# Jimmy2027/MoPoE-MIMIC

Hardware: AMD Instinct MI355X
Metric: samples/sec (higher is better)
Workload: dtype f32; 1 GPU; BASELINE config c2: MoPoE joint-ELBO train step, 3 modalities (PA+Lateral+text) 128x128, class_dim 128, DIM_img 64, DIM_text 128, vocab 3517, batch 64/GPU, fp32 (storage, accumulation and every product; where the launch plan says so the fp32 products are formed on the bf16 matrix pipe from exact three-way splits of both operands -- closer to fp64 than the fp32 MFMA, tests: test_f32_products_on_the; global_batch=64, parallelism=dp1, hip_graph=True, cross_rank_elbo=mean

## Files before the change

include/mopoe_hip.h:

```cpp
#ifndef MOPOE_HIP_H
#define MOPOE_HIP_H

#include <stddef.h>
#include <stdint.h>

#ifdef __cplusplus
extern "C" {
#endif

#define MOPOE_ABI_VERSION 23

#define MOPOE_OK 0
#define MOPOE_ERR_ARG (-1)
#define MOPOE_ERR_LAUNCH (-2)
#define MOPOE_ERR_DEVICE (-3)

int mopoe_abi_version(void);
const char* mopoe_last_error(void);

typedef struct {
  int32_t N;
  int32_t Hs, Ws;
  int32_t Hb, Wb;
  int32_t Cin, Cout;
// ... 150 lines not shown
                               const mopoe_mask_ref* mask1, const double* sums2, double* sums1, float* dw1, float* dbias,
                               float* dgamma2, float* dbeta2, void* stream);
int mopoe_block_front_stats(const float* x, const float* w1, const float* bias, int64_t rows, int32_t C,
                            const mopoe_bn_ref* bn1, const mopoe_mask_ref* mask1, double* stats_d1, void* stream);
int mopoe_block_front_apply(const float* x, const float* w1, const float* bias, float* a2, int64_t rows, int32_t C,
                            const mopoe_bn_ref* bn1, const mopoe_bn_ref* bn2, const mopoe_mask_ref* mask1, void* stream);
int mopoe_block_front_bwd(const float* x, const float* dh2, const float* w1, const float* bias, float* dh1, int64_t rows, int32_t C,
                          const mopoe_bn_ref* bn1, const mopoe_bn_ref* bn2, const mopoe_mask_ref* mask1, const double* sums2,
                          double* sums1, float* dw1, float* dbias, float* dgamma2, float* dbeta2, void* stream);
int mopoe_lse_rows(const void* logits, int32_t is_bf16, int64_t rows, int32_t V, float* lse, void* stream);
int mopoe_token_nll_logits_fwd(const void* logits, int32_t is_bf16, const float* lse, const float* ids, int64_t rows, int32_t V,
                               float norm, float* out, double* ws, void* stream);
int mopoe_token_softmax_grad_logits(const void* logits, int32_t is_bf16, const float* lse, const float* ids, const float* g,
                                    int64_t rows, int32_t V, float norm, void* dx, void* stream);
int mopoe_dense_logprob_rows(const float* logp, const float* target, int64_t rows, int64_t per_row,
                             int64_t target_rows, float* out, void* stream);

int mopoe_lhood_style_sample(const float* mu, const float* logvar, const float* eps, const float* style_mu,
                             const float* style_logvar, const float* style_eps, int32_t K, int32_t B, int32_t D, int32_t S,
                             float* zcat, float* t_c, float* t_s, void* stream);
int mopoe_lhood_estimates(const float* const lp[3], const float* t_c, const float* t_s, int32_t K, int32_t B,
                          int32_t subset_mask, float* out, void* stream);

int mopoe_logreg_fit(const float* X, const float* Y, int32_t S, int32_t N, int32_t D, int32_t L, float C, int32_t max_iter,
                     float tol, float* W, float* info, void* stream);
int mopoe_logreg_predict(const float* const* x, int32_t S, int32_t M, int32_t D, int32_t L, const float* W, float* pred,
                         float* dec, void* stream);

int mopoe_embedding_fwd(const float* ids, const float* table, float* out, int64_t rows, int32_t V,
                        int32_t D, void* stream);
int mopoe_embedding_bwd(const float* ids, const float* gout, float* dtable, int64_t rows, int32_t V,
                        int32_t D, int32_t padding_idx, void* stream);


int mopoe_conv_fwd_bf16(const uint16_t* x, const uint16_t* wp, const float* bias, void* y, int32_t y_is_f32,
                        const mopoe_conv_geom* g, const mopoe_bn_ref* bn_in, const mopoe_mask_ref* mask,
                        double* out_stats, const mopoe_conv_plan* plan, void* workspace, size_t workspace_bytes,
                        void* stream);
int mopoe_conv_fwd_mix_bf16(const uint16_t* x, const uint16_t* wp, const float* bias, uint16_t* y,
                            const mopoe_conv_geom* g, const mopoe_bn_ref* bn_in, const mopoe_mask_ref* mask,
                            const mopoe_mix_ref* mix, double* out_stats, const mopoe_conv_plan* plan, void* workspace,
                            size_t workspace_bytes, void* stream);
int mopoe_conv_dgrad_bf16(const uint16_t* dy, const uint16_t* wp, void* dx, int32_t dx_is_f32, const mopoe_conv_geom* g,
                          const mopoe_bn_ref* relu_bn, const uint16_t* xin, double* bwd_sums,
                          const mopoe_conv_plan* plan, void* workspace, size_t workspace_bytes, void* stream);
int mopoe_conv_wgrad_bf16(const uint16_t* x, const uint16_t* dy, float* dwp, const mopoe_conv_geom* g,
                          const mopoe_bn_ref* bn_in, int32_t dwp_is_zero, const mopoe_conv_plan* plan, void* stream);
int mopoe_edge_expand_bf16(const float* scal, const float* w, uint16_t* out, const mopoe_conv_geom* g, int32_t C,
                           double* stats, void* stream);
int mopoe_edge_wgrad_bf16(const uint16_t* vec, const float* scal, float* dw, const mopoe_conv_geom* g, int32_t C,
                          int32_t dw_is_zero, void* stream);
int mopoe_edge_reduce_bf16(const uint16_t* x, const float* w, const float* bias, float* out, const mopoe_conv_geom* g,
                           int32_t C, void* stream);
int mopoe_bn_relu_apply_bf16(const uint16_t* x, uint16_t* out, int64_t rows, int32_t C, const mopoe_bn_ref* bn, void* stream);
int mopoe_block_out_fwd_bf16(const uint16_t* s, const uint16_t* m, uint16_t* out, int64_t rows, int32_t C,
                             const mopoe_bn_ref* bn_s, float a, float b, double* out_stats, void* stream);
int mopoe_bn_bwd_reduce_bf16(const uint16_t* g, const uint16_t* s, int64_t rows, int32_t C, const mopoe_bn_ref* bn_s,
                             double* sums, void* stream);
int mopoe_block_out_bwd_bf16(const uint16_t* g, const uint16_t* s, uint16_t* dm, uint16_t* ds, int64_t rows, int32_t C,
                             const mopoe_bn_ref* bn_s, const double* sums, const mopoe_mask_ref* mask, float a, float b,
                             float* dgamma, float* dbeta, float* colsum_dm, float* colsum_ds, void* stream);
int mopoe_bn_bwd_apply_bf16(const uint16_t* dy, const uint16_t* x, const uint16_t* add, uint16_t* dx, int64_t rows,
                            int32_t C, const mopoe_bn_ref* bn, const double* sums, const mopoe_mask_ref* mask,
                            float* dgamma, float* dbeta, float* colsum_dx, const uint16_t* next_s,
                            const mopoe_bn_ref* next_bn, double* next_sums, void* stream);
int mopoe_colsum_bf16(const uint16_t* x, float* out, int64_t rows, int32_t C, int32_t out_is_zero, void* stream);
int mopoe_logsoftmax_bwd_bf16out(const float* dy, const float* y, uint16_t* dx, int64_t rows, int32_t V, void* stream);
int mopoe_embedding_fwd_bf16(const float* ids, const float* table, uint16_t* out, int64_t rows, int32_t V, int32_t D,
                             void* stream);
int mopoe_embedding_bwd_bf16(const float* ids, const uint16_t* gout, float* dtable, int64_t rows, int32_t V, int32_t D,
                             int32_t padding_idx, void* stream);

typedef struct {
  float* p;
  const float* g;
  float* m;
  float* v;
  uint16_t* p16;
  int64_t n;
} mopoe_adam_seg;
int mopoe_adam_step(const mopoe_adam_seg* segs, int32_t nseg, float* step, const float* lr_dev, double lr, double beta1,
                    double beta2, double eps, float* coef, void* stream);

#define MOPOE_PROF_KINDS 144
int mopoe_prof_enable(int32_t on);
int mopoe_prof_stamp(uint64_t* slot, void* stream);
int mopoe_prof_collect(int64_t* launches, double* total_ms, double* total_flops, double* total_bytes );

#ifdef __cplusplus
}
#endif
#endif
```

mopoe-mimic_amd/csrc/conv_gemm.hip:

```cpp
#include "gemm_common.hpp"

namespace mopoe {

constexpr int BK = 16;
#ifndef TILE_N64_REMAINDER
#define TILE_N64_REMAINDER 64
#endif
#ifndef SPLIT_BLOCKS
#define SPLIT_BLOCKS 256
#endif
#ifndef SPLIT_TARGET
#define SPLIT_TARGET 512
#endif
#ifndef GEMM_8WAVES
#define GEMM_8WAVES 1
#endif
#ifndef PERSIST_BLOCKS
#define PERSIST_BLOCKS 2048
#endif
#ifndef GEMM_MIN_WAVES
#define GEMM_MIN_WAVES 3
#endif
#ifndef GEMM_BK_BIG
#define GEMM_BK_BIG 16
#endif
#ifndef GEMM_LDS_PAD
#define GEMM_LDS_PAD 4
#endif
constexpr int LDS_PAD = GEMM_LDS_PAD;

struct GemmArgs {
  const float* X;
  const float* W;
  float* Y;
  const float* bias;
  int N, Hx, Wx, Hy, Wy, Ck, Cn, Cin_w, Cout_w;
  int kh, kw, sh, sw, ph, pw;
  int form, w_nk;
  int Hq, Wq;
  long rows_per_phase;
  int vecA, vecB;
  mopoe_bn_ref bn_in;
  mopoe_mask_ref mask;
  double* out_stats;
  mopoe_bn_ref relu_bn;
  const float* xin;
  double* bwd_sums;
  unsigned x_bytes, w_bytes;
  int nsplit;
  float* partial;
  int* counters;
  long rows_total;
  int mix;
  float mix_a, mix_b;
  int xcd_remap;
};

__device__ __forceinline__ float epi_round(const GemmArgs&, float x) { return x; }
struct EpiXinRaw { float4 lo, hi; };
constexpr bool EPI_PREFETCH_XIN = false;
__device__ __forceinline__ EpiXinRaw epi_xin_ld(const GemmArgs& a, long yrow, int ncol, bool ok_hi) {
  const float* p = a.xin + yrow * a.Cn + ncol;
  EpiXinRaw r;
  r.lo = *reinterpret_cast<const float4*>(p);
  r.hi = ok_hi ? *reinterpret_cast<const float4*>(p + 4) : make_float4(0.f, 0.f, 0.f, 0.f);
  return r;
}
__device__ __forceinline__ void epi_xin_unpack(const EpiXinRaw& r, float (&xi)[8]) {
  xi[0] = r.lo.x; xi[1] = r.lo.y; xi[2] = r.lo.z; xi[3] = r.lo.w; xi[4] = r.hi.x; xi[5] = r.hi.y; xi[6] = r.hi.z; xi[7] = r.hi.w;
}
__device__ __forceinline__ void epi_store8(const GemmArgs& a, long yrow, int ncol, bool ok_hi, const float (&v)[8]) {
  float* dst = a.Y + yrow * a.Cn + ncol;
  *reinterpret_cast<float4*>(dst) = make_float4(v[0], v[1], v[2], v[3]);
  if (ok_hi) *reinterpret_cast<float4*>(dst + 4) = make_float4(v[4], v[5], v[6], v[7]);
}


__device__ __forceinline__ float4 bld4(__amdgpu_buffer_rsrc_t srd, unsigned byte_off) {
  const u32x4 v = __builtin_amdgcn_raw_buffer_load_b128(srd, byte_off, 0, 0);
  return make_float4(__uint_as_float(v.x), __uint_as_float(v.y), __uint_as_float(v.z), __uint_as_float(v.w));
}

// ... 1092 lines not shown
    return edge_expand(x, wp, y, g, g->Cout, out_stats, (hipStream_t)stream);
  if (plain && g->transposed && g->Cout == 1 && !out_stats && edge_supported(g, g->Cin, {x, wp}))
    return edge_reduce(x, wp, bias, y, g, g->Cin, (hipStream_t)stream);
  return launch_gather(x, wp, bias, y, g, g->transposed ? 0 : 1, g->Cin, g->Cout, 0, bn_in, mask, out_stats,
                       nullptr, nullptr, nullptr, plan, workspace, workspace_bytes, (hipStream_t)stream);
}

extern "C" int mopoe_conv_fwd_mix(const float* x, const float* wp, const float* bias, float* y, const mopoe_conv_geom* g,
                                  const mopoe_bn_ref* bn_in, const mopoe_mask_ref* mask, const mopoe_mix_ref* mix,
                                  double* out_stats, const mopoe_conv_plan* plan, void* workspace, size_t workspace_bytes,
                                  void* stream) {
  if (int rc = validate_geom(g)) return rc;
  if (!x || !wp || !y || !mix) { set_error("conv_fwd_mix: null pointer"); return MOPOE_ERR_ARG; }
  return launch_gather(x, wp, bias, y, g, g->transposed ? 0 : 1, g->Cin, g->Cout, 0, bn_in, mask, out_stats,
                       nullptr, nullptr, nullptr, plan, workspace, workspace_bytes, (hipStream_t)stream, mix);
}

extern "C" int mopoe_conv_dgrad(const float* dy, const float* wp, float* dx, const mopoe_conv_geom* g,
                                const mopoe_bn_ref* relu_bn, const float* xin, double* bwd_sums,
                                const mopoe_conv_plan* plan, void* workspace, size_t workspace_bytes, void* stream) {
  if (int rc = validate_geom(g)) return rc;
  if (!dy || !wp || !dx) { set_error("conv_dgrad: null pointer"); return MOPOE_ERR_ARG; }
  if (g->transposed && g->Cout == 1 && (!relu_bn || relu_bn->mode == 0) && edge_supported(g, g->Cin, {wp, dx}))
    return edge_expand(dy, wp, dx, g, g->Cin, nullptr, (hipStream_t)stream);
  return launch_gather(dy, wp, nullptr, dx, g, g->transposed ? 1 : 0, g->Cout, g->Cin, 1, nullptr, nullptr,
                       nullptr, relu_bn, xin, bwd_sums, plan, workspace, workspace_bytes, (hipStream_t)stream);
}

extern "C" int mopoe_conv_wgrad(const float* x, const float* dy, float* dwp, const mopoe_conv_geom* g,
                                const mopoe_bn_ref* bn_in, int32_t dwp_is_zero, const mopoe_conv_plan* plan,
                                void* stream_) {
  if (int rc = validate_geom(g)) return rc;
  if (!x || !dy || !dwp) { set_error("conv_wgrad: null pointer"); return MOPOE_ERR_ARG; }
  hipStream_t stream = (hipStream_t)stream_;
  if ((!bn_in || bn_in->mode == 0) && !g->transposed && g->Cin == 1 && edge_supported(g, g->Cout, {dy, dwp}))
    return edge_wgrad(dy, x, dwp, g, g->Cout, stream, dwp_is_zero != 0);
  if ((!bn_in || bn_in->mode == 0) && g->transposed && g->Cout == 1 && edge_supported(g, g->Cin, {x, dwp}))
    return edge_wgrad(x, dy, dwp, g, g->Cin, stream, dwp_is_zero != 0);
  WgradArgs a;
  a.Xs = x; a.Dy = dy; a.dW = dwp;
  a.N = g->N; a.Hs = g->Hs; a.Ws = g->Ws; a.Hb = g->Hb; a.Wb = g->Wb; a.Cin = g->Cin; a.Cout = g->Cout;
  a.kh = g->kh; a.kw = g->kw; a.sh = g->sh; a.sw = g->sw; a.ph = g->ph; a.pw = g->pw;
  a.x_is_big = g->transposed ? 0 : 1;
  a.Ms = (long)g->N * g->Hs * g->Ws;
  mopoe_bn_ref none = {};
  a.bn_in = bn_in ? *bn_in : none;
  if (a.bn_in.mode != 0 && (a.bn_in.C != g->Cin || g->Cin > MAX_BN_C)) { set_error("wgrad bn_in channel mismatch"); return MOPOE_ERR_ARG; }
  a.vecI = (g->Cin % 4 == 0) && aligned16(x);
  a.vecJ = (g->Cout % 4 == 0) && aligned16(dy);
  const size_t rows_x = (size_t)g->N * (g->transposed ? g->Hs * g->Ws : g->Hb * g->Wb);
  const size_t rows_dy = (size_t)g->N * (g->transposed ? g->Hb * g->Wb : g->Hs * g->Ws);
  const size_t xb = rows_x * g->Cin * sizeof(float), db = rows_dy * g->Cout * sizeof(float);
  const bool vec = a.vecI && a.vecJ && xb < (1ull << 31) && db < (1ull << 31);
  a.x_bytes = (unsigned)std::min<size_t>(xb, 0x7fffffffu);
  a.dy_bytes = (unsigned)std::min<size_t>(db, 0x7fffffffu);
  if (rows_x >= (1ull << 31) || rows_dy >= (1ull << 31)) { set_error("wgrad: more than 2^31 rows"); return MOPOE_ERR_ARG; }
  const int hw_s = g->Hs * g->Ws;
  a.fast = (vec && ((g->Ws % BK == 0) || (BK % g->Ws == 0 && hw_s % BK == 0))) ? 1 : 0;
  const int taps = g->kh * g->kw;
  bool big = g->Cin > 64 && g->Cout > 64;
  if (plan && (plan->tile == 9 || plan->tile == 10)) {
    const bool ok = a.bn_in.mode == 0 && vec && g->kh == 4 && g->kw == 4 && g->sh == 2 && g->sw == 2 && g->ph == 1 && g->pw == 1 &&
                    g->Hs % 8 == 0 && g->Ws % 8 == 0 && g->Hb == 2 * g->Hs && g->Wb == 2 * g->Ws;
    if (!ok) {
      set_error("wgrad plan: tiles 9 / 10 (four taps per block) need a plain operand, the vector path, k4 s2 p1 and a small grid of whole 8 x 8 tiles");
      return MOPOE_ERR_ARG;
    }
    const int Cg = a.x_is_big ? g->Cin : g->Cout, Csm = a.x_is_big ? g->Cout : g->Cin;
    const int cs = plan->tile == 10 ? 128 : 64;
    if (cs == 128 && Csm % 128 != 0) { set_error("wgrad plan: tile 10 needs a multiple of 128 channels on the small-grid operand (%d)", Csm); return MOPOE_ERR_ARG; }
    const long ntiles = (long)g->N * (g->Hs / 8) * (g->Ws / 8);
    const long cblocks = (long)ceil_div(Cg, 64) * ceil_div(Csm, cs) * 4;
    long split = plan->split > 0 ? plan->split : (256 + cblocks - 1) / cblocks;
    if (split > ntiles) split = ntiles;
    if (split < 1) split = 1;
    a.chunk = (ntiles + split - 1) / split;
    split = (ntiles + a.chunk - 1) / a.chunk;
    a.atomic = split > 1;
    static const bool xcd_remap9 = !getenv("MOPOE_NO_XCD_REMAP");
    a.xcd_remap = xcd_remap9 ? 1 : 0;
    if (a.atomic && !dwp_is_zero) {
      if (hipMemsetAsync(dwp, 0, (size_t)taps * g->Cin * g->Cout * sizeof(float), stream) != hipSuccess) { set_error("wgrad memset failed"); return MOPOE_ERR_LAUNCH; }
    }
    ProfScope prof(stream, 2.0 * (double)a.Ms * g->Cin * (double)g->Cout * taps, PROF_F32_WGRAD_PARITY + (cs == 128 ? 2 : 0) + (a.x_is_big ? 0 : 1), (double)xb + (double)db);
    const dim3 grid((unsigned)(ceil_div(Cg, 64) * ceil_div(Csm, cs)), 4, (unsigned)split);
    if (cs == 128 && a.x_is_big) hipLaunchKernelGGL((wgrad_parity_f32_kernel<128, true>), grid, dim3(256), 0, stream, a);
    else if (cs == 128) hipLaunchKernelGGL((wgrad_parity_f32_kernel<128, false>), grid, dim3(256), 0, stream, a);
    else if (a.x_is_big) hipLaunchKernelGGL((wgrad_parity_f32_kernel<64, true>), grid, dim3(256), 0, stream, a);
    else hipLaunchKernelGGL((wgrad_parity_f32_kernel<64, false>), grid, dim3(256), 0, stream, a);
    return check_launch("wgrad_parity_f32 (four taps per block)");
  }
  const bool wemu = plan && (plan->tile == 7 || plan->tile == 8);
  if (wemu && a.bn_in.mode != 0) { set_error("wgrad plan: tile %d (split-bf16 products) has no BN-on-load form", plan->tile); return MOPOE_ERR_ARG; }
  if (plan && (plan->tile == 2 || plan->tile == 6 || plan->tile == 8)) big = false;
  else if (plan && (plan->tile == 5 || plan->tile == 7)) {
    if (!big) { set_error("wgrad plan: tile %d (128x128 on LDS-DMA) needs more than 64 channels on both sides (%d, %d)", plan->tile, g->Cin, g->Cout); return MOPOE_ERR_ARG; }
  }
  else if (plan && plan->tile > 2) { set_error("wgrad plan: tile %d (see mopoe_conv_plan in mopoe_hip.h: -1, 0, 2, 5, 6, 7, 8, 9, 10)", plan->tile); return MOPOE_ERR_ARG; }
  const bool glds = plan && plan->tile >= 5;
  if (glds && !vec) { set_error("wgrad plan: the LDS-DMA tiles need the vector path (channel counts %% 4 == 0, aligned tensors)"); return MOPOE_ERR_ARG; }
  const int T = big ? 128 : 64;
  const int nI = ceil_div(g->Cin, T), nJ = ceil_div(g->Cout, T);
  a.nJ = nJ;
  const long tiles = (long)nI * nJ * taps;
  long split = (1024 + tiles - 1) / tiles;
  if (plan && plan->split > 0) split = plan->split;
  const int kp = glds ? 32 : BK;
  const long max_split = glds ? (a.Ms + 4 * kp - 1) / (4 * kp) : (a.Ms + 8 * BK - 1) / (8 * BK);
  if (split > max_split) split = max_split;
  if (split < 1) split = 1;
  long chunk = (a.Ms + split - 1) / split;
  chunk = (chunk + kp - 1) / kp * kp;
  split = (a.Ms + chunk - 1) / chunk;
  a.chunk = chunk;
  a.atomic = split > 1;
  static const bool xcd_remap = !getenv("MOPOE_NO_XCD_REMAP");
  a.xcd_remap = xcd_remap ? 1 : 0;
  const size_t bytes = (size_t)taps * g->Cin * g->Cout * sizeof(float);
  if (a.atomic && !dwp_is_zero) {
    if (hipMemsetAsync(dwp, 0, bytes, stream) != hipSuccess) { set_error("wgrad memset failed"); return MOPOE_ERR_LAUNCH; }
  }
  const double flops = 2.0 * (double)a.Ms * g->Cin * (double)g->Cout * taps;
  const int spec = a.fast ? (a.bn_in.mode != 0 ? 2 : 1) : 0;
  const double abytes = ((double)g->N * g->Hs * g->Ws * (g->transposed ? g->Cin : g->Cout)
                         + (double)g->N * g->Hb * g->Wb * (g->transposed ? g->Cout : g->Cin)) * sizeof(float);
  ProfScope prof(stream, flops, wemu ? PROF_F32_WGRAD_GLDS_EMU + (big ? 0 : 1)
                                : glds ? PROF_F32_WGRAD_GLDS + (big ? 0 : 2) + (a.bn_in.mode != 0 ? 1 : 0)
                                     : (vec ? PROF_WGRAD_VEC + (big ? 0 : 3) + spec : PROF_WGRAD_SCALAR + (big ? 0 : 1)), abytes);
  dim3 grid(nI * nJ, taps, (unsigned)split);
  if (wemu) {
    if (big) hipLaunchKernelGGL((wgrad_gemm_f32_glds_kernel<128, false, 2, 1>), grid, dim3(256), 0, stream, a);
    else hipLaunchKernelGGL((wgrad_gemm_f32_glds_kernel<64, false, 4, 1>), grid, dim3(256), 0, stream, a);
  } else if (glds) {
    const bool xf = a.bn_in.mode != 0;
    if (big) {
      if (xf) hipLaunchKernelGGL((wgrad_gemm_f32_glds_kernel<128, true, 2>), grid, dim3(256), 0, stream, a);
      else hipLaunchKernelGGL((wgrad_gemm_f32_glds_kernel<128, false, 2>), grid, dim3(256), 0, stream, a);
    } else {
      if (xf) hipLaunchKernelGGL((wgrad_gemm_f32_glds_kernel<64, true, 2>), grid, dim3(256), 0, stream, a);
      else hipLaunchKernelGGL((wgrad_gemm_f32_glds_kernel<64, false, 4>), grid, dim3(256), 0, stream, a);
    }
  } else if (vec) {
    if (big) {
      if (spec == 1) hipLaunchKernelGGL((wgrad_gemm_kernel<128, 128, true, 1>), grid, dim3(256), 0, stream, a);
      else if (spec == 2) hipLaunchKernelGGL((wgrad_gemm_kernel<128, 128, true, 2>), grid, dim3(256), 0, stream, a);
      else hipLaunchKernelGGL((wgrad_gemm_kernel<128, 128, true, 0>), grid, dim3(256), 0, stream, a);
    } else {
      if (spec == 1) hipLaunchKernelGGL((wgrad_gemm_kernel<64, 64, true, 1>), grid, dim3(256), 0, stream, a);
      else if (spec == 2) hipLaunchKernelGGL((wgrad_gemm_kernel<64, 64, true, 2>), grid, dim3(256), 0, stream, a);
      else hipLaunchKernelGGL((wgrad_gemm_kernel<64, 64, true, 0>), grid, dim3(256), 0, stream, a);
    }
  } else {
    if (big) hipLaunchKernelGGL((wgrad_gemm_kernel<128, 128, false>), grid, dim3(256), 0, stream, a);
    else hipLaunchKernelGGL((wgrad_gemm_kernel<64, 64, false>), grid, dim3(256), 0, stream, a);
  }
  return check_launch("wgrad_gemm");
}
```

mopoe-mimic_amd/csrc/conv_gemm_glds_parity.inc:

```
template <int CS, bool G_IS_A>
__global__ __launch_bounds__(256, 1) __attribute__((amdgpu_waves_per_eu(1, 1))) void wgrad_parity_f32_kernel(const WgradArgs a) {
  static_assert(CS == 64 || CS == 128, "S tile of 64 or 128 channels");
  constexpr int G_ROWB = 256, S_ROWB = CS * 4;
  constexpr int G_PIECES = 24, G_BYTES = G_PIECES * 1024;
  constexpr int S_BYTES = 64 * S_ROWB, S_PIECES = S_BYTES / 1024;
  constexpr int STAGE_BYTES = G_BYTES + S_BYTES;
  constexpr int G_INSTR = G_PIECES / 4, S_INSTR = S_PIECES / 4;
  constexpr int LPS = G_INSTR + S_INSTR;
  constexpr int S_LPR = S_ROWB / 16, S_RPP = 64 / S_LPR;
  constexpr int NSTAGE = CS == 128 ? 2 : 3;
  constexpr int NU = CS == 128 ? 2 : 1;
  constexpr int TJ = 2;
  static_assert(NSTAGE * STAGE_BYTES <= 160 * 1024, "LDS");
  __shared__ __attribute__((aligned(1024))) unsigned char smem[NSTAGE * STAGE_BYTES];

  const int tid = threadIdx.x;
  const int lane = tid & 63, wave = __builtin_amdgcn_readfirstlane(tid >> 6);
  const int wi = wave >> 1;
  const int wj = CS == 128 ? (wave & 1) : 0;
  const int tu0 = CS == 128 ? 0 : (wave & 1);
  const unsigned lin = a.xcd_remap ? xcd_swizzle(blockIdx.x + gridDim.x * (blockIdx.y + gridDim.y * blockIdx.z),
                                                 gridDim.x * gridDim.y * gridDim.z)
                                   : blockIdx.x + gridDim.x * (blockIdx.y + gridDim.y * blockIdx.z);
  const unsigned bx = lin % gridDim.x, byz = lin / gridDim.x;
  const unsigned by = byz % gridDim.y, bz = byz / gridDim.y;
  const int Cg = a.x_is_big ? a.Cin : a.Cout, Csm = a.x_is_big ? a.Cout : a.Cin;
  const int nSt = (Csm + CS - 1) / CS;
  const int g0 = (int)(bx / nSt) * 64, s0 = (int)(bx % nSt) * CS;
  const int py = (int)by >> 1, px = (int)by & 1;
  const int tw = a.Ws >> 3, th = a.Hs >> 3;
  const long ntiles = (long)a.N * th * tw;
  const long tbeg = (long)bz * a.chunk;
  const long tend = tbeg + a.chunk < ntiles ? tbeg + a.chunk : ntiles;
  const int total = (int)(tend > tbeg ? tend - tbeg : 0);

  const float* const Gp = a.x_is_big ? a.Xs : a.Dy;
  const float* const Sp = a.x_is_big ? a.Dy : a.Xs;
  const __amdgpu_buffer_rsrc_t srdG = __builtin_amdgcn_make_buffer_rsrc((void*)Gp, 0, (int)(a.x_is_big ? a.x_bytes : a.dy_bytes), 0x00020000);
  const __amdgpu_buffer_rsrc_t srdS = __builtin_amdgcn_make_buffer_rsrc((void*)Sp, 0, (int)(a.x_is_big ? a.dy_bytes : a.x_bytes), 0x00020000);
  const unsigned lds_base = (unsigned)(uintptr_t)((lds_void_t*)smem);

  int ga[G_INSTR], gb[G_INSTR];
  unsigned gch[G_INSTR];
#pragma unroll
  for (int t = 0; t < G_INSTR; ++t) {
    const int R = 4 * (t * 4 + wave) + (lane >> 4);
    const int ch = g0 + (lane & 15) * 4;
    ga[t] = R / 9;
    gb[t] = R - ga[t] * 9;
    gch[t] = (R < 81 && ch < Cg) ? (unsigned)ch * 4u : OOB;
  }
  int si[S_INSTR], sj[S_INSTR];
  unsigned sch;
  {
    const int ch = s0 + (lane % S_LPR) * 4;
    sch = ch < Csm ? (unsigned)ch * 4u : OOB;
  }
#pragma unroll
  for (int t = 0; t < S_INSTR; ++t) {
    const int k = S_RPP * (t * 4 + wave) + lane / S_LPR;
    si[t] = k >> 3;
    sj[t] = k & 7;
  }

  const int l31 = lane & 31, lhi = lane >> 5;
  unsigned goff[NSTAGE], soff[NSTAGE][TJ];
#pragma unroll
  for (int b = 0; b < NSTAGE; ++b) {
    goff[b] = lds_base + (unsigned)(b * STAGE_BYTES) + (unsigned)(9 * (lhi + tu0)) * G_ROWB + (unsigned)(wi * 32 + l31) * 4u;
#pragma unroll
    for (int j = 0; j < TJ; ++j)
      soff[b][j] = lds_base + (unsigned)(b * STAGE_BYTES + G_BYTES) + (unsigned)(8 * lhi) * S_ROWB + (unsigned)(wj * 64 + j * 32 + l31) * 4u;
  }

  long tile_next = tbeg;
  auto issue = [&](auto bufc) {
    constexpr int buf = decltype(bufc)::value;
    const long t = tile_next++;
    const int n = (int)(t / (th * tw));
    const int rem = (int)(t - (long)n * (th * tw));
    const int oy0 = (rem / tw) * 8, ox0 = (rem % tw) * 8;
    unsigned char* const stage = smem + buf * STAGE_BYTES;
#pragma unroll
    for (int k = 0; k < G_INSTR; ++k) {
      const int iy = 2 * (oy0 + ga[k]) + py - 1, ix = 2 * (ox0 + gb[k]) + px - 1;
      const bool ok = ((unsigned)iy < (unsigned)a.Hb) & ((unsigned)ix < (unsigned)a.Wb) & (gch[k] != OOB);
      const unsigned off = ok ? ((unsigned)((n * a.Hb + iy) * a.Wb + ix) * (unsigned)Cg) * 4u + gch[k] : OOB;
      lds_dma16(srdG, stage + (k * 4 + wave) * 1024, off, 0u);
    }
#pragma unroll
    for (int k = 0; k < S_INSTR; ++k) {
      const unsigned row = (unsigned)((n * a.Hs + oy0 + si[k]) * a.Ws + ox0 + sj[k]);
      const unsigned off = sch != OOB ? row * (unsigned)Csm * 4u + sch : OOB;
      lds_dma16(srdS, stage + G_BYTES + (k * 4 + wave) * 1024, off, 0u);
    }
  };
  auto top = [&](int it, auto curc) {
    constexpr int cur = decltype(curc)::value;
    const int younger = total - 1 - it < NSTAGE - 2 ? total - 1 - it : NSTAGE - 2;
    if (NSTAGE >= 3 && younger == 1) wait_vmcnt<LPS>();
    else wait_vmcnt<0>();
    __builtin_amdgcn_sched_barrier(0);
    __builtin_amdgcn_s_barrier();
    __builtin_amdgcn_sched_barrier(0);
    if (it + NSTAGE - 1 < total) issue(std::integral_constant<int, (cur + NSTAGE - 1) % NSTAGE>{});
  };

  f32x16 acc[NU][2][TJ];
#pragma unroll
  for (int u = 0; u < NU; ++u)
#pragma unroll
    for (int v = 0; v < 2; ++v)
#pragma unroll
      for (int j = 0; j < TJ; ++j)
#pragma unroll
        for (int r = 0; r < 16; ++r) acc[u][v][j][r] = 0.f;

  constexpr int NF = CS == 128 ? 1 : 2;
  float fg[NF][NU][9], fs[NF][TJ][8];
  Split3 sg[2][NU][2], ss[2][TJ];
  unsigned g8h[NU], g8m[NU], g8l[NU];
  float r0 = 0.f, r1 = 0.f;

  auto reads = [&](auto curc, auto sc, auto fc) {
    constexpr int cur = decltype(curc)::value, s = decltype(sc)::value, f = decltype(fc)::value;
    static_for<NU>([&](auto uc) {
      constexpr int u = decltype(uc)::value;
      static_for<9>([&](auto ec) {
        constexpr int e = decltype(ec)::value;
        lds_frag_f1<(18 * s + 9 * u + e) * G_ROWB>(fg[f][u][e], goff[cur]);
      });
    });
#pragma unroll
    for (int j = 0; j < TJ; ++j)
      static_for<8>([&](auto ec) {
        constexpr int e = decltype(ec)::value;
        lds_frag_f1<(16 * s + e) * S_ROWB>(fs[f][j][e], soff[cur][j]);
      });
  };
  auto fence_f = [&](auto fc) {
    constexpr int f = decltype(fc)::value;
    MOPOE_DEVICE_ASM("s_waitcnt lgkmcnt(0)" ::: "memory");
#pragma unroll
    for (int u = 0; u < NU; ++u)
#pragma unroll
      for (int e = 0; e < 9; ++e) pin_reg(fg[f][u][e]);
#pragma unroll
    for (int j = 0; j < TJ; ++j)
#pragma unroll
      for (int e = 0; e < 8; ++e) pin_reg(fs[f][j][e]);
    __builtin_amdgcn_sched_barrier(0);
  };
  constexpr int GU = 12, NG = NU * GU + 16;
  auto group = [&](auto gc, auto fc, auto dc) {
    constexpr int g = decltype(gc)::value, f = decltype(fc)::value, d = decltype(dc)::value;
    if constexpr (g < NU * GU) {
      constexpr int u = g / GU, k = g % GU;
      if constexpr (k < 10) {
        constexpr int w = k / 2;
        if constexpr (k % 2 == 0) {
          unsigned h;
          split3_first(fg[f][u][2 * w], w < 4 ? fg[f][u][w < 4 ? 2 * w + 1 : 0] : 0.f, h, r0, r1);
          if constexpr (w < 4) sg[d][u][0].h[w < 4 ? w : 0] = h; else g8h[u] = h;
        } else {
          unsigned m, l;
          split3_second(r0, r1, m, l);
          if constexpr (w < 4) { sg[d][u][0].m[w < 4 ? w : 0] = m; sg[d][u][0].l[w < 4 ? w : 0] = l; } else { g8m[u] = m; g8l[u] = l; }
        }
      } else {
        static_for<2>([&](auto xc) {
          constexpr int w = 2 * (k - 10) + decltype(xc)::value;
          const unsigned nh = w < 3 ? sg[d][u][0].h[w < 3 ? w + 1 : 0] : g8h[u], nm = w < 3 ? sg[d][u][0].m[w < 3 ? w + 1 : 0] : g8m[u],
                         nl = w < 3 ? sg[d][u][0].l[w < 3 ? w + 1 : 0] : g8l[u];
          sg[d][u][1].h[w] = __builtin_amdgcn_alignbit(nh, sg[d][u][0].h[w], 16);
          sg[d][u][1].m[w] = __builtin_amdgcn_alignbit(nm, sg[d][u][0].m[w], 16);
          sg[d][u][1].l[w] = __builtin_amdgcn_alignbit(nl, sg[d][u][0].l[w], 16);
        });
      }
    } else {
      constexpr int k = g - NU * GU, j = k / 8, w = (k % 8) / 2;
      if constexpr (k % 2 == 0) {
        unsigned h;
        split3_first(fs[f][j][2 * w], fs[f][j][2 * w + 1], h, r0, r1);
        ss[d][j].h[w] = h;
      } else {
        unsigned m, l;
        split3_second(r0, r1, m, l);
        ss[d][j].m[w] = m; ss[d][j].l[w] = l;
      }
    }
  };
  constexpr int NACC = NU * 2 * TJ, NM = 6 * NACC;
  auto mfma_t = [&](auto tc, auto dc) {
    constexpr int t = decltype(tc)::value, d = decltype(dc)::value;
    constexpr int term = t / NACC, tile = t % NACC, j = tile % TJ, v = (tile / TJ) % 2, u = tile / (2 * TJ);
    if constexpr (G_IS_A) mfma_split_term<term>(acc[u][v][j], sg[d][u][v], ss[d][j]);
    else mfma_split_term<term>(acc[u][v][j], ss[d][j], sg[d][u][v]);
  };
  auto mfma_and_split = [&](auto dc, auto fc, auto&& mid) {
    constexpr int d = decltype(dc)::value;
    static_for<(NM > NG ? NM : NG)>([&](auto xc) {
      constexpr int x = decltype(xc)::value;
      if constexpr (x < NM) mfma_t(xc, dc);
      if constexpr (x < NG) group(xc, fc, std::integral_constant<int, 1 - d>{});
      __builtin_amdgcn_sched_barrier(0);
      if constexpr (x == NG - 1) { mid(); __builtin_amdgcn_sched_barrier(0); }
    });
  };
  auto nothing = [] {};
  auto mfma_only = [&](auto dc) { static_for<NM>([&](auto tc) { mfma_t(tc, dc); }); };

  using E0 = std::integral_constant<int, 0>; using E1 = std::integral_constant<int, 1>;
  using E2 = std::integral_constant<int, 2>; using E3 = std::integral_constant<int, 3>;
  if (total > 0) {
    issue(E0{});
    if (NSTAGE >= 3 && total > 1) issue(E1{});
    top(0, E0{});
    int it = 0;
    if constexpr (NF == 2) {
      reads(E0{}, E0{}, E0{});
      reads(E0{}, E1{}, E1{});
      fence_f(E0{});
      fence_f(E1{});
      static_for<NG>([&](auto gc) { group(gc, E0{}, E0{}); });
      __builtin_amdgcn_sched_barrier(0);
      auto tile = [&](auto curc) -> bool {
        constexpr int cur = decltype(curc)::value, nxt = (cur + 1) % NSTAGE;
        using NX = std::integral_constant<int, nxt>;
        reads(curc, E2{}, E0{});
        mfma_and_split(E0{}, E1{}, nothing);
        fence_f(E0{});
        reads(curc, E3{}, E1{});
        mfma_and_split(E1{}, E0{}, nothing);
        fence_f(E1{});
        const bool more = it + 1 < total;
        if (more) { top(it + 1, NX{}); reads(NX{}, E0{}, E0{}); }
        mfma_and_split(E0{}, E1{}, nothing);
        if (!more) { mfma_only(E1{}); return true; }
        fence_f(E0{});
        reads(NX{}, E1{}, E1{});
        mfma_and_split(E1{}, E0{}, nothing);
        fence_f(E1{});
        ++it;
        return false;
      };
      while (true) {
        if (tile(E0{})) break;
        if (tile(E1{})) break;
        if constexpr (NSTAGE >= 3) { if (tile(E2{})) break; }
      }
    } else {
      reads(E0{}, E0{}, E0{});
      fence_f(E0{});
      static_for<NG>([&](auto gc) { group(gc, E0{}, E0{}); });
      __builtin_amdgcn_sched_barrier(0);
      reads(E0{}, E1{}, E0{});
      auto tile = [&](auto curc) -> bool {
        constexpr int cur = decltype(curc)::value, nxt = (cur + 1) % NSTAGE;
        using NX = std::integral_constant<int, nxt>;
        fence_f(E0{});
        mfma_and_split(E0{}, E0{}, [&] { reads(curc, E2{}, E0{}); });
        fence_f(E0{});
        mfma_and_split(E1{}, E0{}, [&] { reads(curc, E3{}, E0{}); });
        fence_f(E0{});
        const bool more = it + 1 < total;
        mfma_and_split(E0{}, E0{}, [&] { if (more) { top(it + 1, NX{}); reads(NX{}, E0{}, E0{}); } });
        if (!more) { mfma_only(E1{}); return true; }
        fence_f(E0{});
        mfma_and_split(E1{}, E0{}, [&] { reads(NX{}, E1{}, E0{}); });
        ++it;
        return false;
      };
      while (true) {
        if (tile(E0{})) break;
        if (tile(E1{})) break;
        if constexpr (NSTAGE >= 3) { if (tile(E2{})) break; }
      }
    }
  }

#pragma unroll
  for (int u = 0; u < NU; ++u)
#pragma unroll
    for (int v = 0; v < 2; ++v) {
      const int tap = (py + 2 * (tu0 + u)) * a.kw + px + 2 * v;
#pragma unroll
      for (int j = 0; j < TJ; ++j) {
#pragma unroll
        for (int r = 0; r < 16; ++r) {
          const int m = (r & 3) + 8 * (r >> 2) + 4 * lhi;
          const int gc = g0 + wi * 32 + (G_IS_A ? m : l31);
          const int sc = s0 + wj * 64 + j * 32 + (G_IS_A ? l31 : m);
          if (gc >= Cg || sc >= Csm) continue;
          const int ci = a.x_is_big ? gc : sc, co = a.x_is_big ? sc : gc;
          float* dst = a.dW + ((long)tap * a.Cin + ci) * a.Cout + co;
          if (a.atomic) unsafeAtomicAdd(dst, acc[u][v][j][r]);
          else *dst = acc[u][v][j][r];
        }
      }
    }
}
```

mopoe-mimic_amd/mimic_amd/ops.py:

```python
from __future__ import annotations

import ctypes as C
import os
from dataclasses import dataclass
from functools import lru_cache
from typing import Optional, Sequence

import torch

_HERE = os.path.dirname(os.path.abspath(__file__))
LIB_PATH = os.environ.get("MOPOE_HIP_LIB") or os.path.join(os.path.dirname(_HERE), "csrc", "libmopoe_hip.so")
ABI_VERSION = 23

RES_A, RES_B = 2.0, 0.3
BN_EPS = 1e-5
SUBSET_MASKS = (1, 2, 4, 3, 5, 6, 7)


class MopoeHipError(RuntimeError):
    pass


class _Geom(C.Structure):
    _fields_ = [(n, C.c_int32) for n in
# ... 1067 lines not shown
def lhood_style_sample(mu, logvar, eps, style_mu, style_logvar, style_eps):
    _dev(mu, logvar, eps, style_mu, style_logvar, style_eps)
    b, d = mu.shape
    s = style_mu.shape[1]
    k = eps.shape[0]
    if (logvar.shape != mu.shape or tuple(eps.shape) != (k, b, d) or tuple(style_mu.shape) != (b, s)
            or style_logvar.shape != style_mu.shape or tuple(style_eps.shape) != (k, b, s)):
        raise MopoeHipError("lhood_style_sample: mu/logvar [B,D], eps [K,B,D], style_mu/style_logvar [B,S], style_eps [K,B,S]")
    zcat = torch.empty(k * b, s + d, dtype=torch.float32, device=mu.device)
    t_c = torch.empty(k * b, dtype=torch.float32, device=mu.device)
    t_s = torch.empty_like(t_c)
    _check(lib().mopoe_lhood_style_sample(_p(mu), _p(logvar), _p(eps), _p(style_mu), _p(style_logvar), _p(style_eps),
                                          k, b, d, s, _p(zcat), _p(t_c), _p(t_s), _stream()))
    return zcat, t_c, t_s


def lhood_estimates(lp, t_c, t_s, n_samples: int, subset_mask: int):
    _dev(*lp, t_c, t_s)
    r = t_c.shape[0]
    if r % n_samples or any(t.shape != (r,) for t in (*lp, t_c) + ((t_s,) if t_s is not None else ())):
        raise MopoeHipError("lhood_estimates: every per-row vector must be [K*B]")
    out = torch.empty(4, dtype=torch.float32, device=t_c.device)
    _check(lib().mopoe_lhood_estimates(_ptr3(lp), _p(t_c), _p(t_s), int(n_samples), r // int(n_samples), int(subset_mask),
                                       _p(out), _stream()))
    return out


def logreg_fit(x, y, c: float = 1.0, max_iter: int = 100, tol: float = 1e-5):
    _dev(x, y)
    if (x.dim() != 3 or y.dim() != 2 or y.shape[0] != x.shape[1] or x.dtype != torch.float32 or y.dtype != torch.float32
            or y.device != x.device):
        raise MopoeHipError("logreg_fit: x [S,N,D] float32 and y [N,L] float32 on one device")
    s, n, d = x.shape
    l = y.shape[1]
    w = torch.empty(s, l, d + 1, dtype=torch.float32, device=x.device)
    info = torch.empty(s, l, 2, dtype=torch.float32, device=x.device)
    _check(lib().mopoe_logreg_fit(_p(x), _p(y), s, n, d, l, C.c_float(c), int(max_iter), C.c_float(tol), _p(w), _p(info),
                                  _stream()))
    return w, info


def logreg_predict(x, w, want_decision: bool = False):
    xs = list(x.unbind(0)) if isinstance(x, torch.Tensor) else list(x)
    _dev(w, *xs)
    if (w.dim() != 3 or len(xs) != w.shape[0] or len(xs) > 8 or w.dtype != torch.float32
            or any(t.dim() != 2 or t.shape != xs[0].shape or t.shape[1] + 1 != w.shape[2] or t.dtype != torch.float32
                   or t.device != w.device for t in xs)):
        raise MopoeHipError("logreg_predict: S <= 8 float32 matrices [M,D] and w [S,L,D+1] float32 on one device")
    s, l = w.shape[0], w.shape[1]
    m, d = xs[0].shape
    pred = torch.empty(s, m, l, dtype=torch.float32, device=w.device)
    dec = torch.empty_like(pred) if want_decision else None
    ptrs = (C.c_void_p * s)(*[t.data_ptr() for t in xs])
    _check(lib().mopoe_logreg_predict(ptrs, s, m, d, l, _p(w), _p(pred), _p(dec), _stream()))
    return (pred, dec) if want_decision else pred


def embedding_fwd(ids, table, out_dtype=None):
    _dev(ids, table)
    out_dtype = out_dtype or torch.float32
    out = torch.empty(*ids.shape, table.shape[1], dtype=out_dtype, device=table.device)
    fn = lib().mopoe_embedding_fwd_bf16 if out_dtype == BF16 else lib().mopoe_embedding_fwd
    _check(fn(_p(ids), _p(table), _p(out), C.c_int64(ids.numel()), table.shape[0], table.shape[1], _stream()))
    return out


def embedding_bwd(ids, gout, vocab, padding_idx=0):
    _dev(ids, gout)
    dtable = torch.empty(vocab, gout.shape[-1], dtype=torch.float32, device=gout.device)
    fn = lib().mopoe_embedding_bwd_bf16 if _is16(gout) else lib().mopoe_embedding_bwd
    _check(fn(_p(ids), _p(gout), _p(dtable), C.c_int64(ids.numel()), vocab, gout.shape[-1], padding_idx, _stream()))
    return dtable


def prof_enable(on: bool):
    _check(lib().mopoe_prof_enable(int(on)))


_TILE_TEMPLATES = ("128, 128, 2, 4, 16", "256, 64, 4, 2, 16", "64, 64, 2, 2, 16", "256, 128, 4, 2, 16", "128, 64, 2, 2, 16",
                   "64, 64, 2, 2, 32", "128, 64, 2, 2, 32", "128, 128, 2, 2, 16")


def _prof_kind_names():
    names = [None] * 144
    names[140], names[141] = "wgrad_parity_f32_kernel<64, true>", "wgrad_parity_f32_kernel<64, false>"
    names[142], names[143] = "wgrad_parity_f32_kernel<128, true>", "wgrad_parity_f32_kernel<128, false>"
    names[138], names[139] = "wgrad_gemm_f32_glds_kernel<128, false, 2, 1>", "wgrad_gemm_f32_glds_kernel<64, false, 4, 1>"
    for i, tt in enumerate(("128, 128, 2, 2, {}, 2, 1, 1", "128, 64, 2, 1, {}, 3, 2, 1", "64, 64, 2, 1, {}, 4, 2, 1", "256, 128, 4, 2, {}, 3, 1, 1")):
        for k, spec in enumerate((1, 3)):
            names[130 + 2 * i + k] = f"gather_gemm_f32_glds_kernel<{tt.format(spec)}>"
    names[127], names[128], names[129] = "pw_front_fwd_f32_kernel<false>", "pw_front_fwd_f32_kernel<true>", "pw_front_bwd_f32_kernel"
    names[124], names[125], names[126] = "pw_front_fwd_bf16_kernel<64, false>", "pw_front_fwd_bf16_kernel<64, true>", "pw_front_bwd_bf16_kernel<64>"
    names[122], names[123] = "wgrad_parity_bf16_kernel<64, *>", "wgrad_parity_bf16_kernel<128, *>"
    for m in (1, 2):
        names[120 + m - 1] = f"wgrad_gemm_bf16_glds_kernel<128, false, true, {m}>"
    for i, (tt, st) in enumerate((("128", (2, 2)), ("64", (4, 2)))):
        for xf in (0, 1):
            names[116 + 2 * i + xf] = f"wgrad_gemm_f32_glds_kernel<{tt}, {'true' if xf else 'false'}, {st[xf]}, 0>"
    for i, tt in enumerate(("128, 128, 2, 2, {}, 2, 1, 0", "128, 64, 2, 2, {}, 3, 1, 0", "64, 64, 2, 2, {}, 4, 1, 0", "256, 128, 4, 2, {}, 2, 1, 0")):
        for spec in (1, 2, 3):
            names[104 + 3 * i + spec - 1] = f"gather_gemm_f32_glds_kernel<{tt.format(spec)}>"
    for i, tt in enumerate(("128", "64")):
        for xf in (0, 1):
            names[100 + 2 * i + xf] = f"wgrad_gemm_bf16_glds_kernel<{tt}, {'true' if xf else 'false'}, true, 0>"
    for i, tt in enumerate(("128, 128, 2, 2, 2, 2", "256, 128, 4, 2, 2, 2", "128, 64, 4, 1, 2, 2")):
        names[94 + i] = f"gather_gemm_bf16_glds_kernel<{tt}>"
    names[98] = "gather_gemm_bf16_glds_kernel<64, 64, 2, 2, 2, 4>"
    for i, tt in enumerate(("128, 128, 2, 2, {}, 2", "128, 128, 2, 2, {}, 3", "256, 128, 4, 2, {}, 2", "256, 128, 4, 2, {}, 3",
                            "128, 64, 4, 1, {}, 2", "128, 64, 4, 1, {}, 3", "64, 64, 2, 2, {}, 4")):
        for k, spec in enumerate((1, 3)):
            names[80 + 2 * i + k] = f"gather_gemm_bf16_glds_kernel<{tt.format(spec)}>"
    for tile, tt in enumerate(("128, 128, 2, 2", "256, 64, 4, 1", "64, 64, 2, 2", "256, 128, 4, 2", "128, 64, 4, 1")):
        for spec in (1, 2, 3):
            names[60 + tile * 3 + spec - 1] = f"gather_gemm_bf16_kernel<{tt}, {spec}>"
    for i, tt in enumerate(("128, 128", "64, 64")):
        for xf in (0, 1):
            names[75 + 2 * i + xf] = f"wgrad_gemm_bf16_kernel<{tt}, {'true' if xf else 'false'}, true>"
    for tile, tt in enumerate(_TILE_TEMPLATES):
        for spec in range(4):
            names[tile * 4 + spec] = f"gather_gemm_kernel<{tt}, true, {spec}>"
    for i, tt in enumerate(("128, 128, 2, 2, 16", "256, 64, 4, 1, 16", "64, 64, 2, 2, 16")):
        names[32 + i] = f"gather_gemm_kernel<{tt}, false, 0>"
    for i, tt in enumerate(("128, 128", "64, 64")):
        for spec in range(3):
            names[36 + 3 * i + spec] = f"wgrad_gemm_kernel<{tt}, true, {spec}>"
        names[42 + i] = f"wgrad_gemm_kernel<{tt}, false, 0>"
    for i, tt in enumerate(("2, 2, 2, 2", "4, 1, 2, 2", "2, 2, 1, 1", "2, 1, 2, 2")):
        for spec in range(1, 4):
            names[44 + 4 * i + spec] = f"direct_gemm_kernel<{tt}, {spec}>"
    return names


PROF_KINDS = _prof_kind_names()


def prof_collect():
    k = len(PROF_KINDS)
    n, ms, fl, by = (C.c_int64 * k)(), (C.c_double * k)(), (C.c_double * k)(), (C.c_double * k)()
    _check(lib().mopoe_prof_collect(n, ms, fl, by))
    return {name: (n[i], ms[i], fl[i], by[i]) for i, name in enumerate(PROF_KINDS) if name is not None and n[i] > 0}
```

Before: 6611 samples/sec.

## Add K-partitioned form of the 64-channel parity wgrad kernel with LDS reduction

Adds a K-partitioned variant of the four-tap parity f32 wgrad kernel for 64-channel S tiles. Previously the two waves of a pair each took a different tap row. Now each wave accumulates both tap rows over half of the reduction rows, so each S fragment load and split feeds twice as many MFMAs. The two partial sums are combined through an LDS exchange that overlays the operand stages before the store. It is selected by default when the per-block tile chunk is at least 8, and an env var forces either form. The cost is doubled accumulator registers per wave and an extra barrier-synchronised reduction at the end.

```diff
diff --git a/include/mopoe_hip.h b/include/mopoe_hip.h
--- a/include/mopoe_hip.h
+++ b/include/mopoe_hip.h
@@ -256,7 +256,7 @@
 int mopoe_adam_step(const mopoe_adam_seg* segs, int32_t nseg, float* step, const float* lr_dev, double lr, double beta1,
                     double beta2, double eps, float* coef, void* stream);
 
-#define MOPOE_PROF_KINDS 144
+#define MOPOE_PROF_KINDS 146
 int mopoe_prof_enable(int32_t on);
 int mopoe_prof_stamp(uint64_t* slot, void* stream);
 int mopoe_prof_collect(int64_t* launches, double* total_ms, double* total_flops, double* total_bytes );
diff --git a/mopoe-mimic_amd/csrc/conv_gemm.hip b/mopoe-mimic_amd/csrc/conv_gemm.hip
--- a/mopoe-mimic_amd/csrc/conv_gemm.hip
+++ b/mopoe-mimic_amd/csrc/conv_gemm.hip
@@ -1,3 +1,5 @@
+#include <string.h>
+
 #include "gemm_common.hpp"
 
 namespace mopoe {
@@ -1256,12 +1258,21 @@
     if (a.atomic && !dwp_is_zero) {
       if (hipMemsetAsync(dwp, 0, (size_t)taps * g->Cin * g->Cout * sizeof(float), stream) != hipSuccess) { set_error("wgrad memset failed"); return MOPOE_ERR_LAUNCH; }
     }
-    ProfScope prof(stream, 2.0 * (double)a.Ms * g->Cin * (double)g->Cout * taps, PROF_F32_WGRAD_PARITY + (cs == 128 ? 2 : 0) + (a.x_is_big ? 0 : 1), (double)xb + (double)db);
+    bool kpart = cs == 64 && a.chunk >= WGRAD9_KPART_MIN_CHUNK;
+    if (const char* form = getenv("MOPOE_WGRAD9_FORM")) {
+      if (!strcmp(form, "taps")) kpart = false;
+      else if (!strcmp(form, "kpart")) kpart = cs == 64;
+      else { set_error("MOPOE_WGRAD9_FORM: 'taps' or 'kpart' (%s)", form); return MOPOE_ERR_ARG; }
+    }
+    ProfScope prof(stream, 2.0 * (double)a.Ms * g->Cin * (double)g->Cout * taps,
+                   PROF_F32_WGRAD_PARITY + (kpart ? 4 : cs == 128 ? 2 : 0) + (a.x_is_big ? 0 : 1), (double)xb + (double)db);
     const dim3 grid((unsigned)(ceil_div(Cg, 64) * ceil_div(Csm, cs)), 4, (unsigned)split);
-    if (cs == 128 && a.x_is_big) hipLaunchKernelGGL((wgrad_parity_f32_kernel<128, true>), grid, dim3(256), 0, stream, a);
-    else if (cs == 128) hipLaunchKernelGGL((wgrad_parity_f32_kernel<128, false>), grid, dim3(256), 0, stream, a);
-    else if (a.x_is_big) hipLaunchKernelGGL((wgrad_parity_f32_kernel<64, true>), grid, dim3(256), 0, stream, a);
-    else hipLaunchKernelGGL((wgrad_parity_f32_kernel<64, false>), grid, dim3(256), 0, stream, a);
+    if (cs == 128 && a.x_is_big) hipLaunchKernelGGL((wgrad_parity_f32_kernel<128, true, false>), grid, dim3(256), 0, stream, a);
+    else if (cs == 128) hipLaunchKernelGGL((wgrad_parity_f32_kernel<128, false, false>), grid, dim3(256), 0, stream, a);
+    else if (kpart && a.x_is_big) hipLaunchKernelGGL((wgrad_parity_f32_kernel<64, true, true>), grid, dim3(256), 0, stream, a);
+    else if (kpart) hipLaunchKernelGGL((wgrad_parity_f32_kernel<64, false, true>), grid, dim3(256), 0, stream, a);
+    else if (a.x_is_big) hipLaunchKernelGGL((wgrad_parity_f32_kernel<64, true, false>), grid, dim3(256), 0, stream, a);
+    else hipLaunchKernelGGL((wgrad_parity_f32_kernel<64, false, false>), grid, dim3(256), 0, stream, a);
     return check_launch("wgrad_parity_f32 (four taps per block)");
   }
   const bool wemu = plan && (plan->tile == 7 || plan->tile == 8);
diff --git a/mopoe-mimic_amd/csrc/conv_gemm_glds_parity.inc b/mopoe-mimic_amd/csrc/conv_gemm_glds_parity.inc
--- a/mopoe-mimic_amd/csrc/conv_gemm_glds_parity.inc
+++ b/mopoe-mimic_amd/csrc/conv_gemm_glds_parity.inc
@@ -1,6 +1,8 @@
-template <int CS, bool G_IS_A>
+template <int CS, bool G_IS_A, bool KP>
 __global__ __launch_bounds__(256, 1) __attribute__((amdgpu_waves_per_eu(1, 1))) void wgrad_parity_f32_kernel(const WgradArgs a) {
   static_assert(CS == 64 || CS == 128, "S tile of 64 or 128 channels");
+  static_assert(!KP || CS == 64, "the K-partitioned form is tile 9's");
+  constexpr bool WIDE = CS == 128 || KP;
   constexpr int G_ROWB = 256, S_ROWB = CS * 4;
   constexpr int G_PIECES = 24, G_BYTES = G_PIECES * 1024;
   constexpr int S_BYTES = 64 * S_ROWB, S_PIECES = S_BYTES / 1024;
@@ -9,7 +11,7 @@
   constexpr int LPS = G_INSTR + S_INSTR;
   constexpr int S_LPR = S_ROWB / 16, S_RPP = 64 / S_LPR;
   constexpr int NSTAGE = CS == 128 ? 2 : 3;
-  constexpr int NU = CS == 128 ? 2 : 1;
+  constexpr int NU = WIDE ? 2 : 1;
   constexpr int TJ = 2;
   static_assert(NSTAGE * STAGE_BYTES <= 160 * 1024, "LDS");
   __shared__ __attribute__((aligned(1024))) unsigned char smem[NSTAGE * STAGE_BYTES];
@@ -18,7 +20,8 @@
   const int lane = tid & 63, wave = __builtin_amdgcn_readfirstlane(tid >> 6);
   const int wi = wave >> 1;
   const int wj = CS == 128 ? (wave & 1) : 0;
-  const int tu0 = CS == 128 ? 0 : (wave & 1);
+  const int tu0 = WIDE ? 0 : (wave & 1);
+  const int kh = KP ? (wave & 1) : 0;
   const unsigned lin = a.xcd_remap ? xcd_swizzle(blockIdx.x + gridDim.x * (blockIdx.y + gridDim.y * blockIdx.z),
                                                  gridDim.x * gridDim.y * gridDim.z)
                                    : blockIdx.x + gridDim.x * (blockIdx.y + gridDim.y * blockIdx.z);
@@ -64,13 +67,18 @@
   }
 
   const int l31 = lane & 31, lhi = lane >> 5;
-  unsigned goff[NSTAGE], soff[NSTAGE][TJ];
+  constexpr int NGB = KP ? NU : 1;
+  unsigned goff[NSTAGE][NGB], soff[NSTAGE][TJ];
 #pragma unroll
   for (int b = 0; b < NSTAGE; ++b) {
-    goff[b] = lds_base + (unsigned)(b * STAGE_BYTES) + (unsigned)(9 * (lhi + tu0)) * G_ROWB + (unsigned)(wi * 32 + l31) * 4u;
+#pragma unroll
+    for (int ub = 0; ub < NGB; ++ub) {
+      const int urow = KP ? (ub ^ kh) : tu0;
+      goff[b][ub] = lds_base + (unsigned)(b * STAGE_BYTES) + (unsigned)(18 * kh + 9 * (lhi + urow)) * G_ROWB + (unsigned)(wi * 32 + l31) * 4u;
+    }
 #pragma unroll
     for (int j = 0; j < TJ; ++j)
-      soff[b][j] = lds_base + (unsigned)(b * STAGE_BYTES + G_BYTES) + (unsigned)(8 * lhi) * S_ROWB + (unsigned)(wj * 64 + j * 32 + l31) * 4u;
+      soff[b][j] = lds_base + (unsigned)(b * STAGE_BYTES + G_BYTES) + (unsigned)(16 * kh + 8 * lhi) * S_ROWB + (unsigned)(wj * 64 + j * 32 + l31) * 4u;
   }
 
   long tile_next = tbeg;
@@ -116,7 +124,7 @@
 #pragma unroll
         for (int r = 0; r < 16; ++r) acc[u][v][j][r] = 0.f;
 
-  constexpr int NF = CS == 128 ? 1 : 2;
+  constexpr int NF = WIDE ? 1 : 2;
   float fg[NF][NU][9], fs[NF][TJ][8];
   Split3 sg[2][NU][2], ss[2][TJ];
   unsigned g8h[NU], g8m[NU], g8l[NU];
@@ -128,7 +136,7 @@
       constexpr int u = decltype(uc)::value;
       static_for<9>([&](auto ec) {
         constexpr int e = decltype(ec)::value;
-        lds_frag_f1<(18 * s + 9 * u + e) * G_ROWB>(fg[f][u][e], goff[cur]);
+        lds_frag_f1<(18 * s + (KP ? 0 : 9 * u) + e) * G_ROWB>(fg[f][u][e], goff[cur][KP ? u : 0]);
       });
     });
 #pragma unroll
@@ -217,7 +225,30 @@
     if (NSTAGE >= 3 && total > 1) issue(E1{});
     top(0, E0{});
     int it = 0;
-    if constexpr (NF == 2) {
+    if constexpr (KP) {
+      reads(E0{}, E0{}, E0{});
+      fence_f(E0{});
+      static_for<NG>([&](auto gc) { group(gc, E0{}, E0{}); });
+      __builtin_amdgcn_sched_barrier(0);
+      reads(E0{}, E2{}, E0{});
+      auto tile = [&](auto curc) -> bool {
+        constexpr int cur = decltype(curc)::value, nxt = (cur + 1) % NSTAGE;
+        using NX = std::integral_constant<int, nxt>;
+        fence_f(E0{});
+        const bool more = it + 1 < total;
+        mfma_and_split(E0{}, E0{}, [&] { if (more) { top(it + 1, NX{}); reads(NX{}, E0{}, E0{}); } });
+        if (!more) { mfma_only(E1{}); return true; }
+        fence_f(E0{});
+        mfma_and_split(E1{}, E0{}, [&] { reads(NX{}, E2{}, E0{}); });
+        ++it;
+        return false;
+      };
+      while (true) {
+        if (tile(E0{})) break;
+        if (tile(E1{})) break;
+        if (tile(E2{})) break;
+      }
+    } else if constexpr (NF == 2) {
       reads(E0{}, E0{}, E0{});
       reads(E0{}, E1{}, E1{});
       fence_f(E0{});
@@ -279,11 +310,51 @@
     }
   }
 
-#pragma unroll
-  for (int u = 0; u < NU; ++u)
+  if constexpr (KP) {
+    constexpr int X_BYTES = 2 * TJ * 4096;
+    static_assert(4 * X_BYTES <= NSTAGE * STAGE_BYTES, "the exchange slots overlay the operand stages");
+    const unsigned x_own = lds_base + (unsigned)(wave * X_BYTES) + (unsigned)lane * 16u;
+    const unsigned x_partner = lds_base + (unsigned)((wave ^ 1) * X_BYTES) + (unsigned)lane * 16u;
+    wait_vmcnt<0>();
+    MOPOE_DEVICE_ASM("s_waitcnt lgkmcnt(0)" ::: "memory");
+    __builtin_amdgcn_sched_barrier(0);
+    __builtin_amdgcn_s_barrier();
+    __builtin_amdgcn_sched_barrier(0);
+#pragma unroll
+    for (int v = 0; v < 2; ++v)
+#pragma unroll
+      for (int j = 0; j < TJ; ++j)
+#pragma unroll
+        for (int g = 0; g < 4; ++g)
+          lds_store_b128(x_own + (unsigned)(((v * TJ + j) * 4 + g) * 1024),
+                         u32x4{__float_as_uint(acc[1][v][j][4 * g]), __float_as_uint(acc[1][v][j][4 * g + 1]),
+                               __float_as_uint(acc[1][v][j][4 * g + 2]), __float_as_uint(acc[1][v][j][4 * g + 3])});
+    MOPOE_DEVICE_ASM("s_waitcnt lgkmcnt(0)" ::: "memory");
+    __builtin_amdgcn_sched_barrier(0);
+    __builtin_amdgcn_s_barrier();
+    __builtin_amdgcn_sched_barrier(0);
+#pragma unroll
+    for (int v = 0; v < 2; ++v)
+#pragma unroll
+      for (int j = 0; j < TJ; ++j) {
+        u32x4 t0, t1, t2, t3;
+        lds_load_x4(t0, t1, t2, t3, x_partner + (unsigned)((v * TJ + j) * 4096));
+#pragma unroll
+        for (int e = 0; e < 4; ++e) {
+          acc[0][v][j][e] += __uint_as_float(t0[e]);
+          acc[0][v][j][4 + e] += __uint_as_float(t1[e]);
+          acc[0][v][j][8 + e] += __uint_as_float(t2[e]);
+          acc[0][v][j][12 + e] += __uint_as_float(t3[e]);
+        }
+      }
+  }
+
+  constexpr int NUS = KP ? 1 : NU;
+#pragma unroll
+  for (int u = 0; u < NUS; ++u)
 #pragma unroll
     for (int v = 0; v < 2; ++v) {
-      const int tap = (py + 2 * (tu0 + u)) * a.kw + px + 2 * v;
+      const int tap = (py + 2 * (KP ? kh : tu0 + u)) * a.kw + px + 2 * v;
 #pragma unroll
       for (int j = 0; j < TJ; ++j) {
 #pragma unroll
@@ -300,3 +371,5 @@
       }
     }
 }
+
+constexpr int WGRAD9_KPART_MIN_CHUNK = 8;
diff --git a/mopoe-mimic_amd/mimic_amd/ops.py b/mopoe-mimic_amd/mimic_amd/ops.py
--- a/mopoe-mimic_amd/mimic_amd/ops.py
+++ b/mopoe-mimic_amd/mimic_amd/ops.py
@@ -1173,9 +1173,10 @@
 
 
 def _prof_kind_names():
-    names = [None] * 144
-    names[140], names[141] = "wgrad_parity_f32_kernel<64, true>", "wgrad_parity_f32_kernel<64, false>"
-    names[142], names[143] = "wgrad_parity_f32_kernel<128, true>", "wgrad_parity_f32_kernel<128, false>"
+    names = [None] * 146
+    names[140], names[141] = "wgrad_parity_f32_kernel<64, true, false>", "wgrad_parity_f32_kernel<64, false, false>"
+    names[142], names[143] = "wgrad_parity_f32_kernel<128, true, false>", "wgrad_parity_f32_kernel<128, false, false>"
+    names[144], names[145] = "wgrad_parity_f32_kernel<64, true, true>", "wgrad_parity_f32_kernel<64, false, true>"
     names[138], names[139] = "wgrad_gemm_f32_glds_kernel<128, false, 2, 1>", "wgrad_gemm_f32_glds_kernel<64, false, 4, 1>"
     for i, tt in enumerate(("128, 128, 2, 2, {}, 2, 1, 1", "128, 64, 2, 1, {}, 3, 2, 1", "64, 64, 2, 1, {}, 4, 2, 1", "256, 128, 4, 2, {}, 3, 1, 1")):
         for k, spec in enumerate((1, 3)):
```

After: 6616 samples/sec (median of 2 runs). Within noise of the previous version (+0.1%).
